# BigHippo123/pointcloud-raster

Measured on AMD Instinct MI355X. Metric: Mpts/s ingest->finalize, higher is better.
Workload: dtype f32

## Files before the change

pointcloud-raster_amd/csrc/engine.hip:

```cpp
#include "engine.hpp"

#include <cstdlib>
#include <map>
#include <mutex>
#include <new>
#include <vector>

using namespace pcrhip;

namespace {

struct SharedScratch {
    std::mutex borrow_mu;
    std::mutex mu;
    pcr_hip_arena* arena = nullptr;
    hipEvent_t last = nullptr;
    bool has_last = false;
    uint64_t borrows = 0, grows = 0;
    struct Taps {
        int K = -1, r = -1;
        float sx = 0.f, sy = 0.f;
        float* d = nullptr;
        size_t cap = 0;
        std::vector<float> host;
    } taps;
};
constexpr int kMaxDevices = 64;
SharedScratch g_scratch[kMaxDevices];

}

namespace pcrhip {

int ensure_scratch(pcr_hip_engine* e, size_t bytes) {
    PCR_REQUIRE(e->device >= 0 && e->device < kMaxDevices, "scratch: device ordinal out of range");
    SharedScratch& sp = g_scratch[e->device];
    const bool fresh = !e->scratch_borrowed;
    if (fresh) sp.borrow_mu.lock();
    std::lock_guard<std::mutex> lock(sp.mu);
    auto bail = [&](int rc) { if (fresh) sp.borrow_mu.unlock(); return rc; };
    if (!sp.last && hipEventCreateWithFlags(&sp.last, hipEventDisableTiming) != hipSuccess)
        return bail(fail(PCR_HIP_CUDA_ERROR, "scratch: cannot create the hand-over event"));
    size_t cap = 0;
    if (sp.arena) (void)pcr_hip_arena_stats(sp.arena, &cap, nullptr, nullptr);
    if (bytes > cap) {
        if (hipDeviceSynchronize() != hipSuccess) return bail(fail(PCR_HIP_CUDA_ERROR, "scratch: device synchronize failed"));
        if (sp.arena) (void)pcr_hip_arena_destroy(sp.arena);
        sp.arena = nullptr;
        sp.has_last = false;
        int rc = pcr_hip_arena_create(&sp.arena, bytes + bytes / 8);
        if (rc) return bail(rc);
        ++sp.grows;
    }
    void* base = nullptr;
    (void)pcr_hip_arena_reset(sp.arena);
    int rc = pcr_hip_arena_alloc(sp.arena, bytes, &base);
    if (rc) return bail(rc);
    if (fresh) {
        if (sp.has_last && hipStreamWaitEvent(e->stream, sp.last, 0) != hipSuccess)
            return bail(fail(PCR_HIP_CUDA_ERROR, "scratch: cannot order after the previous borrower"));
        ++sp.borrows;
    }
    (void)pcr_hip_arena_stats(sp.arena, &cap, nullptr, nullptr);
    e->d_scratch = static_cast<char*>(base);
    e->scratch_cap = cap;
    e->scratch_borrowed = true;
    return PCR_HIP_OK;
}

int shared_taps(pcr_hip_engine* e, int K, int r, float sx, float sy,
                void (*fill)(std::vector<float>&, int, int, float, float), const float** d_taps, size_t* count) {
    PCR_REQUIRE(e->scratch_borrowed, "shared_taps: the scratch must be borrowed");
    auto& t = g_scratch[e->device].taps;
    if (!(t.d && t.K == K && t.r == r && t.sx == sx && t.sy == sy)) {
        PCR_HIP_TRY(hipStreamSynchronize(e->stream));
        std::vector<float> next;
        fill(next, K, r, sx, sy);
        if (next.size() > t.cap) {
            PCR_HIP_TRY(hipDeviceSynchronize());
            if (t.d) (void)hipFree(t.d);
            t.d = nullptr;
            t.cap = 0;
            PCR_HIP_TRY(hipMalloc(reinterpret_cast<void**>(&t.d), next.size() * sizeof(float)));
            t.cap = next.size();
// ... 40 lines not shown

namespace {

struct DeviceGuard {
    int prev = -1;
    bool changed = false;
    explicit DeviceGuard(int dev) {
        if (hipGetDevice(&prev) == hipSuccess && prev != dev) changed = hipSetDevice(dev) == hipSuccess;
    }
    ~DeviceGuard() { if (changed) (void)hipSetDevice(prev); }
    DeviceGuard(const DeviceGuard&) = delete;
    DeviceGuard& operator=(const DeviceGuard&) = delete;
};

int check_planes(uint32_t mask, const pcr_hip_planes* p, uint32_t allowed, PlanesDev& out) {
    PCR_REQUIRE(p != nullptr, "scatter: null planes");
    PCR_REQUIRE(mask != 0 && (mask & ~allowed) == 0, "scatter: plane mask not supported for this glyph");
    PCR_REQUIRE(!(mask & PCR_HIP_PLANE_SUM) || p->d_sum, "scatter: SUM plane requested but d_sum is null");
    PCR_REQUIRE(!(mask & PCR_HIP_PLANE_WGT) || p->d_wgt, "scatter: WGT plane requested but d_wgt is null");
    PCR_REQUIRE(!(mask & PCR_HIP_PLANE_MAX) || p->d_max, "scatter: MAX plane requested but d_max is null");
    PCR_REQUIRE(!(mask & PCR_HIP_PLANE_MIN) || p->d_min, "scatter: MIN plane requested but d_min is null");
    out.sum = p->d_sum; out.wgt = p->d_wgt; out.mx = p->d_max; out.mn = p->d_min;
    return PCR_HIP_OK;
}

int begin_scatter(pcr_hip_engine* e, uint64_t n) {
    e->stats.points_in = n;
    e->stats.points_valid = 0;
    e->stats.lds_tile_w = e->stats.lds_tile_h = e->stats.lds_apron = e->stats.num_bins = 0;
    e->stats_scatter_chunk = 0;
    e->counters_published = false;
    return PCR_HIP_OK;
}

int begin_published(pcr_hip_engine* e) {
    if (!e->counters_clean) {
        PCR_HIP_TRY(hipMemsetAsync(e->d_counters, 0, 8 * sizeof(unsigned long long), e->stream));
        e->counters_clean = true;
    }
    e->publish_counters = true;
    return PCR_HIP_OK;
}

}

namespace pcrhip {

int fill_identity(pcr_hip_engine* e, uint32_t mask, const PlanesDev& pl) {
    ScopedKernelTimer t(e, "k_state_init");
    const int64_t cells = (int64_t)e->gd.st_rows * e->gd.W;
    int rc = PCR_HIP_OK;
    if ((mask & PCR_HIP_PLANE_SUM) && (rc = pcr_hip_plane_fill(pl.sum, 0.0f, cells, e->stream)) != PCR_HIP_OK) return rc;
    if ((mask & PCR_HIP_PLANE_WGT) && (rc = pcr_hip_plane_fill(pl.wgt, 0.0f, cells, e->stream)) != PCR_HIP_OK) return rc;
    if ((mask & PCR_HIP_PLANE_MAX) && (rc = pcr_hip_plane_fill(pl.mx, -FLT_MAX, cells, e->stream)) != PCR_HIP_OK) return rc;
    if ((mask & PCR_HIP_PLANE_MIN) && (rc = pcr_hip_plane_fill(pl.mn, FLT_MAX, cells, e->stream)) != PCR_HIP_OK) return rc;
    return rc;
}

}

extern "C" {

int pcr_hip_engine_create(pcr_hip_engine** out, const pcr_hip_grid* g, size_t scratch_bytes, pcr_hip_stream s) {
    PCR_REQUIRE(out, "engine_create: null out pointer");
    *out = nullptr;
    int rc = validate_grid(g);
    if (rc) return rc;
    auto* e = new (std::nothrow) pcr_hip_engine();
    if (!e) return fail(PCR_HIP_OUT_OF_MEMORY, "engine_create: host allocation failed");
    e->grid = *g;
    e->gd = make_grid_dev(*g);
    e->stream = static_cast<hipStream_t>(s);
    e->max_bins = kMaxBins;
    if (const char* dbg = std::getenv("PCR_HIP_DEBUG_MAX_BINS")) {
        const int v = std::atoi(dbg);
        if (v >= 1 && v < kMaxBins) e->max_bins = v;
    }
    if (const char* dbg = std::getenv("PCR_HIP_DEBUG_TWO_LEVEL")) e->two_level = std::atoi(dbg) != 0;
    hipError_t err = hipGetDevice(&e->device);
    hipDeviceProp_t prop;
    if (err == hipSuccess) err = hipGetDeviceProperties(&prop, e->device);
    if (err == hipSuccess) {
        e->num_cus = prop.multiProcessorCount > 0 ? prop.multiProcessorCount : 256;
        e->ntiles = e->gd.tiles_x * e->gd.tiles_y;
        err = hipMalloc(reinterpret_cast<void**>(&e->d_touched), (size_t)e->ntiles * sizeof(uint32_t));
    }
    const size_t count_bytes = ((size_t)kVirtualXcds * kMaxBins + kMaxTiles) * sizeof(unsigned);
    if (err == hipSuccess) err = hipMalloc(reinterpret_cast<void**>(&e->d_counters), 16 * sizeof(unsigned long long));
    if (err == hipSuccess) err = hipMalloc(reinterpret_cast<void**>(&e->d_bin_counts), count_bytes);
    if (err == hipSuccess) err = hipMemsetAsync(e->d_touched, 0, (size_t)e->ntiles * sizeof(uint32_t), e->stream);
    if (err == hipSuccess) err = hipMemsetAsync(e->d_counters, 0, 16 * sizeof(unsigned long long), e->stream);
    if (err == hipSuccess) err = hipMemsetAsync(e->d_bin_counts, 0, count_bytes, e->stream);
    e->counts_clean = e->counters_clean = err == hipSuccess;
    if (err == hipSuccess && scratch_bytes) {
        if (ensure_scratch(e, scratch_bytes) != PCR_HIP_OK) err = hipErrorOutOfMemory;
        else release_scratch(e);
    }
    if (err != hipSuccess) {
        std::string msg = std::string("engine_create: ") + hipGetErrorString(err);
        pcr_hip_engine_destroy(e);
        return fail(err == hipErrorOutOfMemory ? PCR_HIP_OUT_OF_MEMORY : PCR_HIP_CUDA_ERROR, msg);
    }
    *out = e;
    return PCR_HIP_OK;
}

int pcr_hip_engine_destroy(pcr_hip_engine* e) {
    if (!e) return PCR_HIP_OK;
    DeviceGuard dev(e->device);
    (void)hipStreamSynchronize(e->stream);
    for (auto& p : e->pending) { (void)hipEventDestroy(p.a); (void)hipEventDestroy(p.b); }
    if (e->d_touched) (void)hipFree(e->d_touched);
    if (e->d_counters) (void)hipFree(e->d_counters);
    if (e->d_bin_counts) (void)hipFree(e->d_bin_counts);
    delete e;
    return PCR_HIP_OK;
}

int pcr_hip_device_scratch_stats(int device, size_t* capacity, size_t* high_water, uint64_t* borrows, uint64_t* grows) {
    PCR_REQUIRE(device >= 0 && device < kMaxDevices, "device_scratch_stats: device ordinal out of range");
    SharedScratch& sp = g_scratch[device];
    std::lock_guard<std::mutex> lock(sp.mu);
    size_t cap = 0, hw = 0;
    if (sp.arena) (void)pcr_hip_arena_stats(sp.arena, &cap, nullptr, &hw);
    if (capacity) *capacity = cap;
    if (high_water) *high_water = hw;
    if (borrows) *borrows = sp.borrows;
    if (grows) *grows = sp.grows;
    return PCR_HIP_OK;
}

int pcr_hip_engine_set_path(pcr_hip_engine* e, int path) {
    PCR_REQUIRE(e, "engine_set_path: null engine");
    PCR_REQUIRE(path >= 0 && path <= 3,
                "engine_set_path: path must be 0 (auto), 1 (direct), 2 (binned) or 3 (moments, Gaussian only)");
    e->forced_path = path;
    return PCR_HIP_OK;
}

int pcr_hip_engine_planes_fresh(pcr_hip_engine* e, int fresh) {
    PCR_REQUIRE(e, "engine_planes_fresh: null engine");
    PCR_REQUIRE(fresh >= 0 && fresh <= 2, "engine_planes_fresh: 0 (accumulate), 1 (identity-filled) or 2 (undefined) expected");
    e->planes_fresh = fresh;
    return PCR_HIP_OK;
}

int pcr_hip_engine_finalize_with_scatter(pcr_hip_engine* e, int n_out, const int* rtypes, float* const* d_outs,
                                         uint32_t* d_bands_done) {
    PCR_REQUIRE(e, "engine_finalize_with_scatter: null engine");
    e->fused_outs.n = 0;
    e->fused_done = nullptr;
    if (n_out == 0) return PCR_HIP_OK;
    PCR_REQUIRE(rtypes && d_outs && d_bands_done, "engine_finalize_with_scatter: null argument");
    PCR_REQUIRE(n_out >= 1 && n_out <= PCR_HIP_MAX_FINALIZE_OUTPUTS, "engine_finalize_with_scatter: 1..8 outputs");
    for (int i = 0; i < n_out; ++i) {
        PCR_REQUIRE(rtypes[i] >= PCR_HIP_SUM && rtypes[i] <= PCR_HIP_COUNT, "pipeline: unknown reduction type");
        PCR_REQUIRE(d_outs[i] && (reinterpret_cast<uintptr_t>(d_outs[i]) & 15) == 0,
                    "engine_finalize_with_scatter: bands must be non-null and 16-byte aligned");
        e->fused_outs.rtype[i] = rtypes[i];
        e->fused_outs.out[i] = d_outs[i];
    }
    e->fused_outs.n = n_out;
    e->fused_done = d_bands_done;
    return PCR_HIP_OK;
}

// ... 200 lines not shown
```

pointcloud-raster_amd/csrc/engine.hpp:

```cpp
#pragma once

#include "common.hpp"

#include <functional>
#include <map>
#include <vector>

struct pcr_hip_engine {
    pcr_hip_grid grid{};
    pcrhip::GridDev gd{};
    hipStream_t stream = nullptr;
    int device = 0;
    int num_cus = 256;

    uint32_t* d_touched = nullptr;
    int ntiles = 0;
    unsigned long long* d_counters = nullptr;

    unsigned* d_bin_counts = nullptr;
    bool counts_clean = false;
    bool counters_clean = false;
    bool publish_counters = false;
    bool counters_published = false;

    int forced_path = 0;
    int max_bins = 0;
    int stats_scatter_chunk = 0;
    bool two_level = true;
    pcr_hip_scatter_stats stats{};
    int planes_fresh = 0;

    pcrhip::FinalizeOuts fused_outs{};
    uint32_t* fused_done = nullptr;
    bool fused_taken = false;

    bool profiling = false;
    std::string profile_only;
    struct Pending { const char* name; hipEvent_t a, b; };
    std::vector<Pending> pending;
    std::map<std::string, std::pair<uint32_t, double>> kernel_ms;

    char* d_scratch = nullptr;
    size_t scratch_cap = 0;
    bool scratch_borrowed = false;
};

namespace pcrhip {

int ensure_scratch(pcr_hip_engine* e, size_t bytes);
void allow_dynamic_lds(const pcr_hip_engine* e, const void* kernel, size_t bytes);
int zero_counters(pcr_hip_engine* e);
void release_scratch(pcr_hip_engine* e);
int shared_taps(pcr_hip_engine* e, int K, int r, float sx, float sy,
                void (*fill)(std::vector<float>&, int, int, float, float), const float** d_taps, size_t* count);

struct ScopedKernelTimer {
    pcr_hip_engine* e;
    const char* name;
    hipEvent_t a = nullptr, b = nullptr;
    ScopedKernelTimer(pcr_hip_engine* eng, const char* nm) : e(eng), name(nm) {
        if (!e->profiling) return;
        if (!e->profile_only.empty() && e->profile_only != nm) return;
        if (hipEventCreate(&a) != hipSuccess || hipEventCreate(&b) != hipSuccess) { a = b = nullptr; return; }
        (void)hipEventRecord(a, e->stream);
    }
    ~ScopedKernelTimer() {
        if (!a) return;
        (void)hipEventRecord(b, e->stream);
        e->pending.push_back({name, a, b});
    }
};

struct BinGeom {
    int tile_w, tile_h;
    int bins_x, bins_y, nbins;
    int chunk;
    int row0, rows;
    int sup_shift;
};
constexpr int kMaxBands = 32;
struct BinItem {
    unsigned bin, first, count, shared;
};
struct TailFill {
    const unsigned* n_items;
    void* plane[4];
    unsigned bits[4];
    long long n16;
};
struct BinBuffers {
    const uint2* records;
    const BinItem* items;
    const unsigned* n_items;
    int max_items;
    void* extra;
    bool fill_folded;
// ... 69 lines not shown
```

pointcloud-raster_amd/csrc/scatter_binned.hip:

```cpp
#include "engine.hpp"

#include <cstdlib>

using namespace pcrhip;

namespace {

constexpr int kThreads = 1024;
constexpr unsigned kLcellMask = (1u << kLcellBits) - 1;
constexpr unsigned kPointItemRecords = 1u << 17;

struct Routed {
    bool valid;
    int bin;
    unsigned lcell;
    int row, col;
};

__device__ __forceinline__ Routed route(const GridDev& g, const BinGeom& b, double wx, double wy) {
    Routed r;
    r.valid = world_to_cell(g, wx, wy, r.col, r.row);
    r.valid = r.valid && r.row >= g.own_r0 && r.row < g.own_r1;
    int sr = r.row - g.st_r0 - b.row0;
    int bx = fast_div(r.col, b.tile_w), by = fast_div(sr, b.tile_h);
// ... 386 lines not shown
    if (blockIdx.x >= *n_items) return;
    const BinItem it = items[blockIdx.x];
    const int tps = 1 << sup_shift;
    for (int i = threadIdx.x; i < tps; i += kThreads) lds_u32[i] = 0;
    __syncthreads();
    const unsigned tile0 = it.bin << sup_shift;
    const uint2* r = rec + it.first;
    for (unsigned j = threadIdx.x; j < it.count; j += kThreads) atomicAdd(&lds_u32[(r[j].x >> kLcellBits) - tile0], 1u);
    __syncthreads();
    for (int i = threadIdx.x; i < tps; i += kThreads) {
        const unsigned c = lds_u32[i];
        if (c) atomicAdd(&tile_count[tile0 + i], c);
    }
}

__global__ void __launch_bounds__(kThreads)
k_sub_scatter(int sup_shift, const uint2* __restrict__ rec, const BinItem* __restrict__ items,
              const unsigned* __restrict__ n_items, unsigned* __restrict__ cursor, uint2* __restrict__ out) {
    extern __shared__ unsigned char lds_raw[];
    if (blockIdx.x >= *n_items) return;
    const BinItem it = items[blockIdx.x];
    const int tps = 1 << sup_shift;
    uint2* stage = reinterpret_cast<uint2*>(lds_raw);
    unsigned* hist = reinterpret_cast<unsigned*>(lds_raw + (size_t)kSubPer * kThreads * sizeof(uint2));
    unsigned* loff = hist + tps;
    unsigned* gbase = loff + tps;
    __shared__ unsigned wave_tot[kThreads / 64];
    for (int i = threadIdx.x; i < tps; i += kThreads) hist[i] = 0;
    __syncthreads();
    const unsigned tile0 = it.bin << sup_shift;
    const uint2* r = rec + it.first;
    uint2 rc[kSubPer];
    unsigned rank[kSubPer];
#pragma unroll
    for (int k = 0; k < kSubPer; ++k) {
        const unsigned j = k * kThreads + threadIdx.x;
        rc[k] = j < it.count ? r[j] : make_uint2(0xFFFFFFFFu, 0u);
    }
#pragma unroll
    for (int k = 0; k < kSubPer; ++k) {
        rank[k] = 0;
        if (rc[k].x != 0xFFFFFFFFu) rank[k] = atomicAdd(&hist[(rc[k].x >> kLcellBits) - tile0], 1u);
    }
    __syncthreads();
    const int per = (tps + kThreads - 1) / kThreads;
    const int lo = threadIdx.x * per, hi = min(lo + per, tps);
    unsigned s = 0;
    for (int i = lo; i < hi; ++i) s += hist[i];
    unsigned incl = s;
    const int lane = threadIdx.x & 63, wave = threadIdx.x >> 6;
#pragma unroll
    for (int off = 1; off < 64; off <<= 1) {
        unsigned t = __shfl_up(incl, off, 64);
        if (lane >= off) incl += t;
    }
    if (lane == 63) wave_tot[wave] = incl;
    __syncthreads();
    unsigned run = incl - s;
    for (int w = 0; w < wave; ++w) run += wave_tot[w];
    for (int i = lo; i < hi; ++i) {
        loff[i] = run;
        run += hist[i];
    }
    for (int i = threadIdx.x; i < tps; i += kThreads) {
        const unsigned c = hist[i];
        if (c) gbase[i] = atomicAdd(&cursor[tile0 + i], c);
    }
    __syncthreads();
#pragma unroll
    for (int k = 0; k < kSubPer; ++k)
        if (rc[k].x != 0xFFFFFFFFu) stage[loff[(rc[k].x >> kLcellBits) - tile0] + rank[k]] = rc[k];
    __syncthreads();
    for (unsigned j = threadIdx.x; j < it.count; j += kThreads) {
        const uint2 q = stage[j];
        const unsigned t = (q.x >> kLcellBits) - tile0;
        out[gbase[t] + (j - loff[t])] = make_uint2(q.x & kLcellMask, q.y);
    }
}

inline int tile_cell_bytes(unsigned mask) {
    return ((mask & 1) ? 8 : 0) + ((mask & 2) ? 4 : 0) + ((mask & 4) ? 4 : 0) + ((mask & 8) ? 4 : 0);
}

inline BinGeom point_bin_geom(const GridDev& g, uint32_t mask) {
    BinGeom b{};
    b.tile_w = 128;
    b.tile_h = std::min(128, (150 * 1024 / (std::max(tile_cell_bytes(mask), 4) * 128)) & ~7);
    b.bins_x = (g.W + b.tile_w - 1) / b.tile_w;
    b.bins_y = (g.st_rows + b.tile_h - 1) / b.tile_h;
    b.nbins = b.bins_x * b.bins_y;
    b.rows = g.st_rows;
    return b;
}

template <unsigned MASK, bool FUSED>
__global__ void __launch_bounds__(kThreads)
k_tile_accum(GridDev g, BinGeom b, PlanesDev pl, const uint2* __restrict__ records,
             const BinItem* __restrict__ items, const unsigned* __restrict__ n_items, int fresh,
             FinalizeOuts fo, const uint32_t* __restrict__ touched, uint32_t* __restrict__ done) {
    extern __shared__ double lds_tile[];
    if (FUSED && blockIdx.x == 0 && threadIdx.x == 0) *done = (fresh == 2 && n_items[1] == 0u) ? 1u : 0u;
    if (blockIdx.x >= *n_items) return;
    const bool full = fresh == 2 && n_items[1] == 0u;
    const BinItem it = items[blockIdx.x];
    const int cells = b.tile_w * b.tile_h;
    double* t_sum = lds_tile;
    unsigned* t_wgt = reinterpret_cast<unsigned*>(t_sum + ((MASK & 1) ? cells : 0));
    float* t_max = reinterpret_cast<float*>(t_wgt + ((MASK & 2) ? cells : 0));
    float* t_min = t_max + ((MASK & 4) ? cells : 0);

    constexpr int kUnroll = 4;
    const uint2* rec = records + it.first;
    uint2 cur[kUnroll], nxt[kUnroll];
    auto fetch = [&](uint2 (&r)[kUnroll], unsigned j0) {
#pragma unroll
        for (int u = 0; u < kUnroll; ++u) {
            const unsigned j = j0 + u * kThreads;
            r[u] = j < it.count ? stream_load(rec + j) : make_uint2(0xFFFFFFFFu, 0u);
        }
    };
    fetch(cur, threadIdx.x);

    for (int i = threadIdx.x; i < cells; i += kThreads) {
        if (MASK & 1) t_sum[i] = 0.0;
        if (MASK & 2) t_wgt[i] = 0u;
        if (MASK & 4) t_max[i] = -FLT_MAX;
        if (MASK & 8) t_min[i] = FLT_MAX;
    }
    __syncthreads();

    for (unsigned j0 = threadIdx.x; j0 < it.count; j0 += kUnroll * kThreads) {
        fetch(nxt, j0 + kUnroll * kThreads);
#pragma unroll
        for (int u = 0; u < kUnroll; ++u) {
            if (cur[u].x == 0xFFFFFFFFu) continue;
            float val = __uint_as_float(cur[u].y);
            if (MASK & 1) unsafeAtomicAdd(&t_sum[cur[u].x], (double)val);
            if (MASK & 2) atomicAdd(&t_wgt[cur[u].x], 1u);
            if (MASK & 4) atomic_max_f32(&t_max[cur[u].x], val);
            if (MASK & 8) atomic_min_f32(&t_min[cur[u].x], val);
        }
#pragma unroll
        for (int u = 0; u < kUnroll; ++u) cur[u] = nxt[u];
    }
    __syncthreads();

    const int bx = it.bin % b.bins_x, by = it.bin / b.bins_x;
    const int c0 = bx * b.tile_w, r0 = b.row0 + by * b.tile_h;
    const int w = min(b.tile_w, g.W - c0), h = min(b.tile_h, b.row0 + b.rows - r0);
    const bool vec = !it.shared && (g.W % 4 == 0) && (w % 4 == 0) &&
                     ((((MASK & 1) ? reinterpret_cast<uintptr_t>(pl.sum) : 0) | ((MASK & 2) ? reinterpret_cast<uintptr_t>(pl.wgt) : 0) |
                       ((MASK & 4) ? reinterpret_cast<uintptr_t>(pl.mx) : 0) | ((MASK & 8) ? reinterpret_cast<uintptr_t>(pl.mn) : 0)) & 15) == 0;
    if (vec) {
        const int qrow = b.tile_w >> 2;
        for (int i = threadIdx.x; i < qrow * h; i += kThreads) {
            int ly = i / qrow, lx = (i - ly * qrow) << 2;
            if (lx >= w) continue;
            int64_t cell = (int64_t)(r0 + ly) * g.W + (c0 + lx);
            int li = ly * b.tile_w + lx;
            float4 a1, a2, a4, a8, g1, g2, g4, g8;
            bool n1 = false, n2 = false, n4 = false, n8 = false;
            if (MASK & 1) {
                double2 lo = *reinterpret_cast<const double2*>(t_sum + li), hi = *reinterpret_cast<const double2*>(t_sum + li + 2);
                a1 = make_float4((float)lo.x, (float)lo.y, (float)hi.x, (float)hi.y);
                n1 = (lo.x != 0.0) | (lo.y != 0.0) | (hi.x != 0.0) | (hi.y != 0.0);
            }
            if (MASK & 2) {
                uint4 c = *reinterpret_cast<const uint4*>(t_wgt + li);
                a2 = make_float4((float)c.x, (float)c.y, (float)c.z, (float)c.w);
                n2 = (c.x | c.y | c.z | c.w) != 0u;
            }
            if (MASK & 4) { a4 = *reinterpret_cast<const float4*>(t_max + li); n4 = (a4.x != -FLT_MAX) | (a4.y != -FLT_MAX) | (a4.z != -FLT_MAX) | (a4.w != -FLT_MAX); }
            if (MASK & 8) { a8 = *reinterpret_cast<const float4*>(t_min + li); n8 = (a8.x != FLT_MAX) | (a8.y != FLT_MAX) | (a8.z != FLT_MAX) | (a8.w != FLT_MAX); }
            if (fresh) {
                if (MASK & 1) g1 = make_float4(0.f, 0.f, 0.f, 0.f);
                if (MASK & 2) g2 = make_float4(0.f, 0.f, 0.f, 0.f);
                if (MASK & 4) g4 = make_float4(-FLT_MAX, -FLT_MAX, -FLT_MAX, -FLT_MAX);
                if (MASK & 8) g8 = make_float4(FLT_MAX, FLT_MAX, FLT_MAX, FLT_MAX);
            } else {
                if ((MASK & 1) && n1) g1 = *reinterpret_cast<const float4*>(pl.sum + cell);
                if ((MASK & 2) && n2) g2 = *reinterpret_cast<const float4*>(pl.wgt + cell);
                if ((MASK & 4) && n4) g4 = *reinterpret_cast<const float4*>(pl.mx + cell);
                if ((MASK & 8) && n8) g8 = *reinterpret_cast<const float4*>(pl.mn + cell);
            }
            typedef float f4v __attribute__((ext_vector_type(4)));
            if (full) n1 = n2 = n4 = n8 = true;
            if ((MASK & 1) && n1) { g1.x += a1.x; g1.y += a1.y; g1.z += a1.z; g1.w += a1.w;
                __builtin_nontemporal_store(f4v{g1.x, g1.y, g1.z, g1.w}, reinterpret_cast<f4v*>(pl.sum + cell)); }
            if ((MASK & 2) && n2) { g2.x += a2.x; g2.y += a2.y; g2.z += a2.z; g2.w += a2.w;
                __builtin_nontemporal_store(f4v{g2.x, g2.y, g2.z, g2.w}, reinterpret_cast<f4v*>(pl.wgt + cell)); }
            if ((MASK & 4) && n4) { g4.x = fmaxf(g4.x, a4.x); g4.y = fmaxf(g4.y, a4.y); g4.z = fmaxf(g4.z, a4.z); g4.w = fmaxf(g4.w, a4.w); *reinterpret_cast<float4*>(pl.mx + cell) = g4; }
            if ((MASK & 8) && n8) { g8.x = fminf(g8.x, a8.x); g8.y = fminf(g8.y, a8.y); g8.z = fminf(g8.z, a8.z); g8.w = fminf(g8.w, a8.w); *reinterpret_cast<float4*>(pl.mn + cell) = g8; }
            if (FUSED && full) {
                const float s4[4] = {g1.x, g1.y, g1.z, g1.w}, w4[4] = {g2.x, g2.y, g2.z, g2.w};
                const float x4[4] = {g4.x, g4.y, g4.z, g4.w}, m4[4] = {g8.x, g8.y, g8.z, g8.w};
                const int trow = ((g.st_r0 + r0 + ly) / g.th) * g.tiles_x;
                bool live[4];
#pragma unroll
                for (int k = 0; k < 4; ++k) live[k] = touched[trow + (c0 + lx + k) / g.tw] != 0u;
                for (int o = 0; o < fo.n; ++o) {
                    float v[4];
#pragma unroll
                    for (int k = 0; k < 4; ++k)
                        v[k] = live[k] ? finalize_rt(fo.rtype[o], (MASK & 1) ? s4[k] : 0.f, (MASK & 2) ? w4[k] : 0.f,
                                                     (MASK & 4) ? x4[k] : -FLT_MAX, (MASK & 8) ? m4[k] : FLT_MAX) : NAN;
                    __builtin_nontemporal_store(f4v{v[0], v[1], v[2], v[3]}, reinterpret_cast<f4v*>(fo.out[o] + cell));
                }
            }
        }
        return;
    }
    for (int i = threadIdx.x; i < b.tile_w * h; i += kThreads) {
        int ly = i / b.tile_w, lx = i - ly * b.tile_w;
        if (lx >= w) continue;
        int64_t cell = (int64_t)(r0 + ly) * g.W + (c0 + lx);
        int li = ly * b.tile_w + lx;
        if (full) {
            if (MASK & 1) pl.sum[cell] = (float)t_sum[li];
            if (MASK & 2) pl.wgt[cell] = (float)t_wgt[li];
            if (MASK & 4) pl.mx[cell] = t_max[li];
            if (MASK & 8) pl.mn[cell] = t_min[li];
        } else if (!it.shared) {
            if (MASK & 1) { double a = t_sum[li]; if (a != 0.0) pl.sum[cell] += (float)a; }
            if (MASK & 2) { unsigned a = t_wgt[li]; if (a) pl.wgt[cell] += (float)a; }
            if (MASK & 4) { float a = t_max[li]; if (a != -FLT_MAX) pl.mx[cell] = fmaxf(pl.mx[cell], a); }
            if (MASK & 8) { float a = t_min[li]; if (a != FLT_MAX) pl.mn[cell] = fminf(pl.mn[cell], a); }
        } else {
            if (MASK & 1) { double a = t_sum[li]; if (a != 0.0) atomic_add_f32(pl.sum + cell, (float)a); }
            if (MASK & 2) { unsigned a = t_wgt[li]; if (a) atomic_add_f32(pl.wgt + cell, (float)a); }
            if (MASK & 4) { float a = t_max[li]; if (a != -FLT_MAX) atomic_max_f32(pl.mx + cell, a); }
            if (MASK & 8) { float a = t_min[li]; if (a != FLT_MAX) atomic_min_f32(pl.mn + cell, a); }
        }
    }
}

__global__ void __launch_bounds__(256)
k_fill_if(const unsigned* __restrict__ n_items, PlanesDev pl, unsigned mask, int64_t cells4) {
    if (n_items[1] == 0u) return;
    const float4 zero = make_float4(0.f, 0.f, 0.f, 0.f), lo = make_float4(-FLT_MAX, -FLT_MAX, -FLT_MAX, -FLT_MAX),
                 hi = make_float4(FLT_MAX, FLT_MAX, FLT_MAX, FLT_MAX);
    const int64_t stride = (int64_t)gridDim.x * 256;
    for (int64_t i = (int64_t)blockIdx.x * 256 + threadIdx.x; i < cells4; i += stride) {
        if (mask & 1) reinterpret_cast<float4*>(pl.sum)[i] = zero;
        if (mask & 2) reinterpret_cast<float4*>(pl.wgt)[i] = zero;
        if (mask & 4) reinterpret_cast<float4*>(pl.mx)[i] = lo;
        if (mask & 8) reinterpret_cast<float4*>(pl.mn)[i] = hi;
    }
}

template <unsigned MASK>
void launch_accum(pcr_hip_engine* e, const GridDev& gd, const BinGeom& b, const PlanesDev& pl, const BinBuffers& bb,
                  bool fused = false) {
    size_t lds = (size_t)b.tile_w * b.tile_h * tile_cell_bytes(MASK);
    auto go = [&](auto kernel, const FinalizeOuts& fo, uint32_t* done) {
        allow_dynamic_lds(e, reinterpret_cast<const void*>(kernel), lds);
        hipLaunchKernelGGL(kernel, dim3(bb.max_items), dim3(kThreads), lds, e->stream, gd, b, pl,
                           bb.records, bb.items, bb.n_items, e->planes_fresh, fo, (const uint32_t*)e->d_touched, done);
    };
    if (fused) go(&k_tile_accum<MASK, true>, e->fused_outs, e->fused_done);
    else go(&k_tile_accum<MASK, false>, FinalizeOuts{}, nullptr);
}

constexpr uint32_t kSelectGeomMask = PCR_HIP_PLANE_SUM;

__global__ void __launch_bounds__(kThreads)
k_tile_select(GridDev g, BinGeom b, unsigned long long* __restrict__ packed, const uint2* __restrict__ records,
              const BinItem* __restrict__ items, const unsigned* __restrict__ n_items, int fresh,
              const unsigned long long* __restrict__ words) {
    extern __shared__ unsigned long long lds_words[];
    if (blockIdx.x >= *n_items) return;
    const bool full = fresh == 2 && n_items[1] == 0u;
    const BinItem it = items[blockIdx.x];
    const int cells = b.tile_w * b.tile_h;

    constexpr int kUnroll = 4;
    const uint2* rec = records + it.first;
    uint2 cur[kUnroll], nxt[kUnroll];
    auto fetch = [&](uint2 (&r)[kUnroll], unsigned j0) {
#pragma unroll
        for (int u = 0; u < kUnroll; ++u) {
            const unsigned j = j0 + u * kThreads;
            r[u] = j < it.count ? stream_load(rec + j) : make_uint2(0xFFFFFFFFu, 0u);
        }
    };
    fetch(cur, threadIdx.x);
    for (int i = threadIdx.x; i < cells; i += kThreads) lds_words[i] = 0ull;
    __syncthreads();

    for (unsigned j0 = threadIdx.x; j0 < it.count; j0 += kUnroll * kThreads) {
        fetch(nxt, j0 + kUnroll * kThreads);
        unsigned long long w[kUnroll];
#pragma unroll
        for (int u = 0; u < kUnroll; ++u) w[u] = cur[u].x != 0xFFFFFFFFu ? words[cur[u].y] : 0ull;
#pragma unroll
        for (int u = 0; u < kUnroll; ++u)
            if (w[u]) atomicMax(&lds_words[cur[u].x], w[u]);
#pragma unroll
        for (int u = 0; u < kUnroll; ++u) cur[u] = nxt[u];
    }
    __syncthreads();

    const int bx = it.bin % b.bins_x, by = it.bin / b.bins_x;
    const int c0 = bx * b.tile_w, r0 = b.row0 + by * b.tile_h;
    const int w = min(b.tile_w, g.W - c0), h = min(b.tile_h, b.row0 + b.rows - r0);
    const bool vec = !it.shared && (g.W % 2 == 0) && (w % 2 == 0) && (reinterpret_cast<uintptr_t>(packed) & 15) == 0;
    if (vec) {
        const int hrow = b.tile_w >> 1;
        for (int i = threadIdx.x; i < hrow * h; i += kThreads) {
            const int ly = i / hrow, lx = (i - ly * hrow) << 1;
            if (lx >= w) continue;
            ulonglong2* dst = reinterpret_cast<ulonglong2*>(packed + (int64_t)(r0 + ly) * g.W + (c0 + lx));
            ulonglong2 a = *reinterpret_cast<const ulonglong2*>(lds_words + ly * b.tile_w + lx);
            if (!full && !(a.x | a.y)) continue;
            if (!fresh) {
                const ulonglong2 cur2 = *dst;
                a.x = a.x > cur2.x ? a.x : cur2.x;
                a.y = a.y > cur2.y ? a.y : cur2.y;
            }
            *dst = a;
        }
        return;
    }
    for (int i = threadIdx.x; i < b.tile_w * h; i += kThreads) {
        const int ly = i / b.tile_w, lx = i - ly * b.tile_w;
        if (lx >= w) continue;
        unsigned long long* dst = packed + (int64_t)(r0 + ly) * g.W + (c0 + lx);
        const unsigned long long a = lds_words[ly * b.tile_w + lx];
        if (full) *dst = a;
        else if (!a) continue;
        else if (it.shared) atomicMax(dst, a);
        else if (fresh) *dst = a;
        else if (a > *dst) *dst = a;
    }
}

template <bool VEC>
// ... 110 lines not shown
    if (rc) return rc;
    char* s = e->d_scratch;
    auto U = [&](size_t o) { return reinterpret_cast<unsigned*>(s + o); };
    BinItem* d_items1 = reinterpret_cast<BinItem*>(s + o_items1);
    uint2* d_rec1 = reinterpret_cast<uint2*>(s + o_rec1);
    PCR_REQUIRE(l1.nbins <= kMaxBins && (!shift || b.nbins <= kMaxTiles), "bin_points: more bins than the count arrays hold");
    unsigned* const d_count1 = e->d_bin_counts;
    unsigned* const d_count2 = e->d_bin_counts + (size_t)nvx * kMaxBins;
    auto scan = [&](int nbins, int vx, unsigned records, unsigned* d_count, size_t o_cursor, size_t o_items, size_t o_nitems, bool every,
                    int publish) {
        ScopedKernelTimer t(e, "k_bin_scan");
        hipLaunchKernelGGL(k_bin_scan, dim3(1), dim3(kThreads), 0, e->stream, nbins, vx, records, d_count, U(o_cursor),
                           reinterpret_cast<BinItem*>(s + o_items), U(o_nitems), every ? 1 : 0, e->d_counters, publish);
    };
    if (!e->counts_clean)
        PCR_HIP_TRY(hipMemsetAsync(e->d_bin_counts, 0, ((size_t)nvx * kMaxBins + kMaxTiles) * sizeof(unsigned), e->stream));
    e->counts_clean = false;
    const int publish = !e->publish_counters ? 0 : e->counters_published ? 2 : 1;
    if (publish) e->counters_clean = false;
    TailFill tf{};
    if (fill && !shift) {
        tf = *fill;
        tf.n_items = U(o_nitems1);
    }
    launch_count(e, gd, l1, full_blocks, x, y, n, U(o_keys), d_count1);
    scan(l1.nbins, nvx, item_records1, d_count1, o_cursor1, o_items1, o_nitems1, every_bin && !shift, publish);
    if (index) launch_bin_scatter<true>(e, l1, nvx, U(o_keys), v, n, U(o_cursor1), d_rec1, tf);
    else launch_bin_scatter<false>(e, l1, nvx, U(o_keys), v, n, U(o_cursor1), d_rec1, tf);
    if (shift) {
        const int tps = 1 << shift;
        {
            ScopedKernelTimer t(e, "k_sub_count");
            hipLaunchKernelGGL(k_sub_count, dim3(max_items1), dim3(kThreads), (size_t)tps * 4, e->stream, shift,
                               d_rec1, d_items1, U(o_nitems1), d_count2);
        }
        scan(b.nbins, 1, item_records, d_count2, o_cursor2, o_items2, o_nitems2, every_bin, 0);
        ScopedKernelTimer t(e, "k_sub_scatter");
        const size_t lds = (size_t)sub_records * sizeof(uint2) + (size_t)tps * 4 * 3;
        allow_dynamic_lds(e, reinterpret_cast<const void*>(&k_sub_scatter), lds);
        hipLaunchKernelGGL(k_sub_scatter, dim3(max_items1), dim3(kThreads), lds, e->stream, shift, d_rec1, d_items1,
                           U(o_nitems1), U(o_cursor2), reinterpret_cast<uint2*>(s + o_rec2));
    }
    PCR_HIP_TRY(hipGetLastError());
    e->counts_clean = true;
    if (publish) e->counters_clean = e->counters_published = true;
    out->fill_folded = tf.n_items != nullptr;
    out->records = reinterpret_cast<uint2*>(s + (shift ? o_rec2 : o_rec1));
    out->items = reinterpret_cast<BinItem*>(s + (shift ? o_items2 : o_items1));
    out->n_items = U(shift ? o_nitems2 : o_nitems1);
    out->max_items = max_items;
    out->extra = extra_bytes ? s + o_extra : nullptr;
    return PCR_HIP_OK;
}

int sweep_passes(const pcr_hip_engine* e, const BinGeom& whole) { return plan_sweep(e, whole).passes; }

int sweep_tiles(pcr_hip_engine* e, const BinGeom& whole, const double* x, const double* y, const float* v, uint64_t n,
                RecordKind kind, unsigned item_records, bool every_bin, size_t extra_bytes, const TilePass& tile_pass,
                const TailFill* fill) {
    const SweepPlan plan = plan_sweep(e, whole);
    if (plan.passes < 1) return -fail(PCR_HIP_INVALID_ARGUMENT, "binned scatter: grid cannot be binned");
    int total_bins = 0;
    for (int pass = 0; pass < plan.passes; ++pass) {
        const int row0 = pass * plan.band_rows, rows = std::min(plan.band_rows, e->gd.st_rows - row0);
        const GridDev gd = band_grid(e->gd, row0, rows);
        if (gd.own_r0 >= gd.own_r1 && !plan.shift) continue;
        BinGeom b = whole;
        b.row0 = row0;
        b.rows = rows;
        b.bins_y = (rows + b.tile_h - 1) / b.tile_h;
        b.nbins = b.bins_x * b.bins_y;
        b.sup_shift = plan.shift;
        total_bins += b.nbins;
        BinBuffers bb{};
        int rc = bin_points(e, gd, b, x, y, v, n, kind, item_records, &bb, every_bin, extra_bytes, fill);
        if (rc == PCR_HIP_OK) rc = tile_pass(gd, b, bb);
        if (rc) return -rc;
    }
    return total_bins;
}

bool binned_point_supported(const pcr_hip_engine* e, uint32_t mask) {
    if (mask == 0 || (mask & ~15u)) return false;
    if (sweep_passes(e, point_bin_geom(e->gd, mask)) < 1) return false;
    uint64_t cells = (uint64_t)e->gd.W * e->gd.st_rows;
    if (e->forced_path != 2 && e->stats.points_in * 16 < cells) return false;
    return e->stats.points_in < (1ull << 32) - (1ull << 20);
}

int binned_point(pcr_hip_engine* e, uint32_t mask, const PlanesDev& pl,
                 const double* x, const double* y, const float* v, uint64_t n) {
    const BinGeom whole = point_bin_geom(e->gd, mask);
    const int64_t cells = (int64_t)e->gd.st_rows * e->gd.W;
    const bool define_all = e->planes_fresh == 2 && sweep_passes(e, whole) == 1 && cells % 4 == 0 &&
                            ((reinterpret_cast<uintptr_t>(pl.sum) | reinterpret_cast<uintptr_t>(pl.wgt) |
                              reinterpret_cast<uintptr_t>(pl.mx) | reinterpret_cast<uintptr_t>(pl.mn)) & 15) == 0;
    if (e->planes_fresh == 2 && !define_all) {
        int rc = fill_identity(e, mask, pl);
        if (rc) return rc;
        e->planes_fresh = 1;
    }
    const bool fused = define_all && e->fused_outs.n > 0 && e->fused_done && e->gd.W % 4 == 0 &&
                       e->gd.own_r0 == e->gd.st_r0 && e->gd.own_r1 - e->gd.own_r0 == e->gd.st_rows;
    TailFill fill{};
    fill.plane[0] = (mask & 1) ? pl.sum : nullptr; fill.bits[0] = 0u;
    fill.plane[1] = (mask & 2) ? pl.wgt : nullptr; fill.bits[1] = 0u;
    fill.plane[2] = (mask & 4) ? pl.mx : nullptr;  fill.bits[2] = 0xFF7FFFFFu;
    fill.plane[3] = (mask & 8) ? pl.mn : nullptr;  fill.bits[3] = 0x7F7FFFFFu;
    fill.n16 = cells / 4;
    const int bins = sweep_tiles(e, whole, x, y, v, n, RecordKind::Value, kPointItemRecords, define_all, 0,
                                 [&](const GridDev& gd, const BinGeom& b, const BinBuffers& bb) {
        if (define_all && !bb.fill_folded)
            hipLaunchKernelGGL(k_fill_if, dim3(2048), dim3(256), 0, e->stream, bb.n_items, pl, mask, cells / 4);
        e->fused_taken = fused;
        ScopedKernelTimer t(e, "k_tile_accum");
        switch (mask) {
#define PCR_ACC(M) case M: launch_accum<M>(e, gd, b, pl, bb, fused); break;
            PCR_ACC(1) PCR_ACC(2) PCR_ACC(3) PCR_ACC(4) PCR_ACC(5) PCR_ACC(6) PCR_ACC(7) PCR_ACC(8)
            PCR_ACC(9) PCR_ACC(10) PCR_ACC(11) PCR_ACC(12) PCR_ACC(13) PCR_ACC(14) PCR_ACC(15)
#undef PCR_ACC
            default: return fail(PCR_HIP_INVALID_ARGUMENT, "scatter_point: empty plane mask");
        }
        return (int)PCR_HIP_OK;
    }, define_all ? &fill : nullptr);
    if (bins < 0) return -bins;
    PCR_HIP_TRY(hipGetLastError());
    set_binned_stats(e, 1, whole.tile_w, whole.tile_h, 0, bins);
    return PCR_HIP_OK;
}

bool binned_select_supported(const pcr_hip_engine* e) { return binned_point_supported(e, kSelectGeomMask); }

int binned_select(pcr_hip_engine* e, unsigned long long* packed, const double* x, const double* y, const float* v,
                  const float* key, uint64_t n) {
    const BinGeom whole = point_bin_geom(e->gd, kSelectGeomMask);
    const int64_t cells = (int64_t)e->gd.st_rows * e->gd.W;
    const bool define_all = e->planes_fresh == 2 && sweep_passes(e, whole) == 1 && cells % 2 == 0 && e->gd.W % 2 == 0 &&
                            (reinterpret_cast<uintptr_t>(packed) & 15) == 0;
    if (e->planes_fresh == 2 && !define_all) {
        ScopedKernelTimer t(e, "k_state_init");
        PCR_HIP_TRY(hipMemsetAsync(packed, 0, (size_t)cells * sizeof(unsigned long long), e->stream));
        e->planes_fresh = 1;
    }
    TailFill fill{};
    fill.plane[0] = packed;
    fill.n16 = cells / 2;
    const int bins = sweep_tiles(e, whole, x, y, nullptr, n, RecordKind::Index, kPointItemRecords, define_all, (size_t)n * 8,
                                 [&](const GridDev& gd, const BinGeom& b, const BinBuffers& bb) {
        if (define_all && !bb.fill_folded)
            hipLaunchKernelGGL(k_zero_if, dim3(2048), dim3(256), 0, e->stream, bb.n_items, packed, cells / 2);
        launch_select(e, gd, b, packed, bb, v, key, n);
        return (int)PCR_HIP_OK;
    }, define_all ? &fill : nullptr);
    if (bins < 0) return -bins;
    PCR_HIP_TRY(hipGetLastError());
    set_binned_stats(e, 1, whole.tile_w, whole.tile_h, 0, bins);
    return PCR_HIP_OK;
}

}
```

Before: 96840.

## Size point tiles to CU count and precompute tile liveness in fused accumulate

Point-bin tile height is now picked by searching heights that minimise rounds-per-CU times height, bounded by the device LDS limit read at engine creation. The fused accumulate kernel gets a dedicated fast path for fresh full bins. It writes planes directly without reading global memory, and it computes per-tile touched flags once through a wave ballot, or through an LDS bitmask when a tile is mixed, instead of per-cell global lookups. Finalize outputs are produced with a branch-free select in place of a per-output finalize_rt call. Taller tiles use more LDS, which may reduce occupancy.

```diff
diff --git a/pointcloud-raster_amd/csrc/engine.hip b/pointcloud-raster_amd/csrc/engine.hip
--- a/pointcloud-raster_amd/csrc/engine.hip
+++ b/pointcloud-raster_amd/csrc/engine.hip
@@ -1,5 +1,6 @@
 #include "engine.hpp"
 
+#include <algorithm>
 #include <cstdlib>
 #include <map>
 #include <mutex>
@@ -206,6 +207,7 @@
     if (err == hipSuccess) err = hipGetDeviceProperties(&prop, e->device);
     if (err == hipSuccess) {
         e->num_cus = prop.multiProcessorCount > 0 ? prop.multiProcessorCount : 256;
+        e->lds_limit = std::max(prop.sharedMemPerBlock, prop.sharedMemPerBlockOptin);
         e->ntiles = e->gd.tiles_x * e->gd.tiles_y;
         err = hipMalloc(reinterpret_cast<void**>(&e->d_touched), (size_t)e->ntiles * sizeof(uint32_t));
     }
diff --git a/pointcloud-raster_amd/csrc/engine.hpp b/pointcloud-raster_amd/csrc/engine.hpp
--- a/pointcloud-raster_amd/csrc/engine.hpp
+++ b/pointcloud-raster_amd/csrc/engine.hpp
@@ -12,6 +12,7 @@
     hipStream_t stream = nullptr;
     int device = 0;
     int num_cus = 256;
+    size_t lds_limit = 64 * 1024;
 
     uint32_t* d_touched = nullptr;
     int ntiles = 0;
diff --git a/pointcloud-raster_amd/csrc/scatter_binned.hip b/pointcloud-raster_amd/csrc/scatter_binned.hip
--- a/pointcloud-raster_amd/csrc/scatter_binned.hip
+++ b/pointcloud-raster_amd/csrc/scatter_binned.hip
@@ -492,11 +492,26 @@
     return ((mask & 1) ? 8 : 0) + ((mask & 2) ? 4 : 0) + ((mask & 4) ? 4 : 0) + ((mask & 8) ? 4 : 0);
 }
 
-inline BinGeom point_bin_geom(const GridDev& g, uint32_t mask) {
+constexpr int kPointTileW = 128;
+inline size_t point_tile_lds(int bytes_per_cell, int h) { return (size_t)kPointTileW * h * bytes_per_cell + (size_t)kPointTileW * h / 8; }
+
+inline BinGeom point_bin_geom(const pcr_hip_engine* e, uint32_t mask) {
+    const GridDev& g = e->gd;
+    const int bytes = std::max(tile_cell_bytes(mask), 4);
     BinGeom b{};
-    b.tile_w = 128;
-    b.tile_h = std::min(128, (150 * 1024 / (std::max(tile_cell_bytes(mask), 4) * 128)) & ~7);
+    b.tile_w = kPointTileW;
     b.bins_x = (g.W + b.tile_w - 1) / b.tile_w;
+    auto bins_of = [&](int h) { return (int64_t)b.bins_x * ((g.st_rows + h - 1) / h); };
+    auto rounds_of = [&](int h) { return (bins_of(h) + e->num_cus - 1) / e->num_cus; };
+    b.tile_h = std::min(128, (150 * 1024 / (bytes * kPointTileW)) & ~7);
+    if (rounds_of(b.tile_h) <= 16) {
+        int64_t best = rounds_of(b.tile_h) * b.tile_h;
+        for (int h = b.tile_h + 8; kPointTileW * h <= (1 << kLcellBits) && point_tile_lds(bytes, h) <= e->lds_limit; h += 8)
+            if (rounds_of(h) * h < best) {
+                best = rounds_of(h) * h;
+                b.tile_h = h;
+            }
+    }
     b.bins_y = (g.st_rows + b.tile_h - 1) / b.tile_h;
     b.nbins = b.bins_x * b.bins_y;
     b.rows = g.st_rows;
@@ -513,11 +528,15 @@
     if (blockIdx.x >= *n_items) return;
     const bool full = fresh == 2 && n_items[1] == 0u;
     const BinItem it = items[blockIdx.x];
-    const int cells = b.tile_w * b.tile_h;
+    const int cells = kPointTileW * b.tile_h;
     double* t_sum = lds_tile;
     unsigned* t_wgt = reinterpret_cast<unsigned*>(t_sum + ((MASK & 1) ? cells : 0));
     float* t_max = reinterpret_cast<float*>(t_wgt + ((MASK & 2) ? cells : 0));
     float* t_min = t_max + ((MASK & 4) ? cells : 0);
+    unsigned* t_live = reinterpret_cast<unsigned*>(t_min + ((MASK & 8) ? cells : 0));
+    const int bx = it.bin % b.bins_x, by = it.bin / b.bins_x;
+    const int c0 = bx * kPointTileW, r0 = b.row0 + by * b.tile_h;
+    const int w = min(kPointTileW, g.W - c0), h = min(b.tile_h, b.row0 + b.rows - r0);
 
     constexpr int kUnroll = 4;
     const uint2* rec = records + it.first;
@@ -530,12 +549,48 @@
         }
     };
     fetch(cur, threadIdx.x);
+
+    unsigned live_all = 0xFu, flag = 0u;
+    bool live_mixed = false;
+    int nt = 0;
+    if (FUSED && full) {
+        const int tr0 = (g.st_r0 + r0) / g.th, tc0 = c0 / g.tw;
+        const int nc = (c0 + w - 1) / g.tw - tc0 + 1, lane = threadIdx.x & 63;
+        nt = ((g.st_r0 + r0 + h - 1) / g.th - tr0 + 1) * nc;
+        if (nt <= 64 && lane < nt) flag = touched[(tr0 + lane / nc) * g.tiles_x + tc0 + lane % nc];
+    }
 
     for (int i = threadIdx.x; i < cells; i += kThreads) {
         if (MASK & 1) t_sum[i] = 0.0;
         if (MASK & 2) t_wgt[i] = 0u;
         if (MASK & 4) t_max[i] = -FLT_MAX;
         if (MASK & 8) t_min[i] = FLT_MAX;
+    }
+
+    if (FUSED && full) {
+        asm volatile("" : "+v"(flag));
+        live_mixed = nt > 64;
+        if (!live_mixed) {
+            const int set = __popcll(__ballot(flag != 0u));
+            live_all = set == nt ? 0xFu : 0u;
+            live_mixed = set != 0 && set != nt;
+        }
+        if (live_mixed)
+            for (int t = threadIdx.x; t < cells / 32; t += kThreads) {
+                const int ly = t >> 2, cb = c0 + ((t & 3) << 5);
+                unsigned bits = 0u;
+                if (ly < h && cb < g.W) {
+                    const uint32_t* trow = touched + ((g.st_r0 + r0 + ly) / g.th) * g.tiles_x;
+                    int tc = cb / g.tw, next = (tc + 1) * g.tw;
+                    unsigned on = trow[tc] != 0u;
+                    const int n = min(32, g.W - cb);
+                    for (int k = 0; k < n; ++k) {
+                        if (cb + k >= next) { ++tc; next += g.tw; on = trow[tc] != 0u; }
+                        bits |= on << k;
+                    }
+                }
+                t_live[t] = bits;
+            }
     }
     __syncthreads();
 
@@ -555,19 +610,98 @@
     }
     __syncthreads();
 
-    const int bx = it.bin % b.bins_x, by = it.bin / b.bins_x;
-    const int c0 = bx * b.tile_w, r0 = b.row0 + by * b.tile_h;
-    const int w = min(b.tile_w, g.W - c0), h = min(b.tile_h, b.row0 + b.rows - r0);
     const bool vec = !it.shared && (g.W % 4 == 0) && (w % 4 == 0) &&
                      ((((MASK & 1) ? reinterpret_cast<uintptr_t>(pl.sum) : 0) | ((MASK & 2) ? reinterpret_cast<uintptr_t>(pl.wgt) : 0) |
                        ((MASK & 4) ? reinterpret_cast<uintptr_t>(pl.mx) : 0) | ((MASK & 8) ? reinterpret_cast<uintptr_t>(pl.mn) : 0)) & 15) == 0;
+    typedef float f4v __attribute__((ext_vector_type(4)));
+    const int lx = (threadIdx.x & 31) << 2, ly0 = threadIdx.x >> 5;
+    if (vec && full) {
+        if (lx >= w || ly0 >= h) return;
+        const int n_out = FUSED ? fo.n : 0;
+        float* band[PCR_HIP_MAX_FINALIZE_OUTPUTS];
+        bool divides = false;
+        unsigned kinds = 0u;
+#pragma unroll
+        for (int o = 0; o < PCR_HIP_MAX_FINALIZE_OUTPUTS; ++o) {
+            band[o] = fo.out[o];
+            kinds |= ((unsigned)fo.rtype[o] & 7u) << (3 * o);
+            divides |= o < n_out && (fo.rtype[o] == PCR_HIP_AVERAGE || fo.rtype[o] == PCR_HIP_WEIGHTED_AVERAGE);
+        }
+        const unsigned vkinds = (unsigned)vector_resident((int)kinds);
+        struct Quad {
+            double2 slo, shi;
+            uint4 cnt;
+            float4 mx, mn;
+            unsigned live;
+        };
+        auto read = [&](int ly) {
+            Quad q{};
+            const int li = ly * kPointTileW + lx;
+            if (MASK & 1) { q.slo = *reinterpret_cast<const double2*>(t_sum + li); q.shi = *reinterpret_cast<const double2*>(t_sum + li + 2); }
+            if (MASK & 2) q.cnt = *reinterpret_cast<const uint4*>(t_wgt + li);
+            if (MASK & 4) q.mx = *reinterpret_cast<const float4*>(t_max + li);
+            if (MASK & 8) q.mn = *reinterpret_cast<const float4*>(t_min + li);
+            q.live = live_all;
+            if (FUSED && live_mixed) q.live = t_live[li >> 5];
+            return q;
+        };
+        const int live_shift = (FUSED && live_mixed) ? (lx & 31) : 0;
+        Quad nq = read(ly0);
+        int64_t cell = (int64_t)(r0 + ly0) * g.W + (c0 + lx);
+        for (int ly = ly0; ly < h; ly += 32, cell += (int64_t)32 * g.W) {
+            const Quad q = nq;
+            if (ly + 32 < h) nq = read(ly + 32);
+            float s4[4] = {0.f, 0.f, 0.f, 0.f}, w4[4] = {0.f, 0.f, 0.f, 0.f};
+            float x4[4] = {-FLT_MAX, -FLT_MAX, -FLT_MAX, -FLT_MAX}, m4[4] = {FLT_MAX, FLT_MAX, FLT_MAX, FLT_MAX};
+            if (MASK & 1) { s4[0] += (float)q.slo.x; s4[1] += (float)q.slo.y; s4[2] += (float)q.shi.x; s4[3] += (float)q.shi.y; }
+            if (MASK & 2) { w4[0] += (float)q.cnt.x; w4[1] += (float)q.cnt.y; w4[2] += (float)q.cnt.z; w4[3] += (float)q.cnt.w; }
+            if (MASK & 4) { x4[0] = fmaxf(x4[0], q.mx.x); x4[1] = fmaxf(x4[1], q.mx.y); x4[2] = fmaxf(x4[2], q.mx.z); x4[3] = fmaxf(x4[3], q.mx.w); }
+            if (MASK & 8) { m4[0] = fminf(m4[0], q.mn.x); m4[1] = fminf(m4[1], q.mn.y); m4[2] = fminf(m4[2], q.mn.z); m4[3] = fminf(m4[3], q.mn.w); }
+            float cnt4[4], avg4[4], max4[4], min4[4];
+            if (FUSED) {
+#pragma unroll
+                for (int k = 0; k < 4; ++k) {
+                    cnt4[k] = w4[k] > 0.0f ? w4[k] : NAN;
+                    avg4[k] = NAN;
+                    max4[k] = x4[k] == -FLT_MAX ? NAN : x4[k];
+                    min4[k] = m4[k] == FLT_MAX ? NAN : m4[k];
+                }
+                if (divides) {
+#pragma unroll
+                    for (int k = 0; k < 4; ++k) avg4[k] = w4[k] > 0.0f ? s4[k] / w4[k] : NAN;
+                }
+            }
+            if (MASK & 1) __builtin_nontemporal_store(f4v{s4[0], s4[1], s4[2], s4[3]}, reinterpret_cast<f4v*>(pl.sum + cell));
+            if (MASK & 2) __builtin_nontemporal_store(f4v{w4[0], w4[1], w4[2], w4[3]}, reinterpret_cast<f4v*>(pl.wgt + cell));
+            if (MASK & 4) *reinterpret_cast<float4*>(pl.mx + cell) = make_float4(x4[0], x4[1], x4[2], x4[3]);
+            if (MASK & 8) *reinterpret_cast<float4*>(pl.mn + cell) = make_float4(m4[0], m4[1], m4[2], m4[3]);
+            if (FUSED) {
+#pragma unroll
+                for (int o = 0; o < PCR_HIP_MAX_FINALIZE_OUTPUTS; ++o) {
+                    if (o >= n_out) break;
+                    const unsigned kind = (vkinds >> (3 * o)) & 7u;
+                    const bool is_sum = kind == PCR_HIP_SUM, is_cnt = kind == PCR_HIP_COUNT, is_max = kind == PCR_HIP_MAX, is_min = kind == PCR_HIP_MIN;
+                    float v[4];
+#pragma unroll
+                    for (int k = 0; k < 4; ++k) {
+                        float f = avg4[k];
+                        f = is_min ? min4[k] : f;
+                        f = is_max ? max4[k] : f;
+                        f = is_cnt ? cnt4[k] : f;
+                        f = is_sum ? s4[k] : f;
+                        v[k] = ((q.live >> (live_shift + k)) & 1u) ? f : NAN;
+                    }
+                    __builtin_nontemporal_store(f4v{v[0], v[1], v[2], v[3]}, reinterpret_cast<f4v*>(band[o] + cell));
+                }
+            }
+        }
+        return;
+    }
     if (vec) {
-        const int qrow = b.tile_w >> 2;
-        for (int i = threadIdx.x; i < qrow * h; i += kThreads) {
-            int ly = i / qrow, lx = (i - ly * qrow) << 2;
-            if (lx >= w) continue;
+        if (lx >= w) return;
+        for (int ly = ly0; ly < h; ly += 32) {
             int64_t cell = (int64_t)(r0 + ly) * g.W + (c0 + lx);
-            int li = ly * b.tile_w + lx;
+            int li = ly * kPointTileW + lx;
             float4 a1, a2, a4, a8, g1, g2, g4, g8;
             bool n1 = false, n2 = false, n4 = false, n8 = false;
             if (MASK & 1) {
@@ -593,30 +727,12 @@
                 if ((MASK & 4) && n4) g4 = *reinterpret_cast<const float4*>(pl.mx + cell);
                 if ((MASK & 8) && n8) g8 = *reinterpret_cast<const float4*>(pl.mn + cell);
             }
-            typedef float f4v __attribute__((ext_vector_type(4)));
-            if (full) n1 = n2 = n4 = n8 = true;
             if ((MASK & 1) && n1) { g1.x += a1.x; g1.y += a1.y; g1.z += a1.z; g1.w += a1.w;
                 __builtin_nontemporal_store(f4v{g1.x, g1.y, g1.z, g1.w}, reinterpret_cast<f4v*>(pl.sum + cell)); }
             if ((MASK & 2) && n2) { g2.x += a2.x; g2.y += a2.y; g2.z += a2.z; g2.w += a2.w;
                 __builtin_nontemporal_store(f4v{g2.x, g2.y, g2.z, g2.w}, reinterpret_cast<f4v*>(pl.wgt + cell)); }
             if ((MASK & 4) && n4) { g4.x = fmaxf(g4.x, a4.x); g4.y = fmaxf(g4.y, a4.y); g4.z = fmaxf(g4.z, a4.z); g4.w = fmaxf(g4.w, a4.w); *reinterpret_cast<float4*>(pl.mx + cell) = g4; }
             if ((MASK & 8) && n8) { g8.x = fminf(g8.x, a8.x); g8.y = fminf(g8.y, a8.y); g8.z = fminf(g8.z, a8.z); g8.w = fminf(g8.w, a8.w); *reinterpret_cast<float4*>(pl.mn + cell) = g8; }
-            if (FUSED && full) {
-                const float s4[4] = {g1.x, g1.y, g1.z, g1.w}, w4[4] = {g2.x, g2.y, g2.z, g2.w};
-                const float x4[4] = {g4.x, g4.y, g4.z, g4.w}, m4[4] = {g8.x, g8.y, g8.z, g8.w};
-                const int trow = ((g.st_r0 + r0 + ly) / g.th) * g.tiles_x;
-                bool live[4];
-#pragma unroll
-                for (int k = 0; k < 4; ++k) live[k] = touched[trow + (c0 + lx + k) / g.tw] != 0u;
-                for (int o = 0; o < fo.n; ++o) {
-                    float v[4];
-#pragma unroll
-                    for (int k = 0; k < 4; ++k)
-                        v[k] = live[k] ? finalize_rt(fo.rtype[o], (MASK & 1) ? s4[k] : 0.f, (MASK & 2) ? w4[k] : 0.f,
-                                                     (MASK & 4) ? x4[k] : -FLT_MAX, (MASK & 8) ? m4[k] : FLT_MAX) : NAN;
-                    __builtin_nontemporal_store(f4v{v[0], v[1], v[2], v[3]}, reinterpret_cast<f4v*>(fo.out[o] + cell));
-                }
-            }
         }
         return;
     }
@@ -661,7 +777,7 @@
 template <unsigned MASK>
 void launch_accum(pcr_hip_engine* e, const GridDev& gd, const BinGeom& b, const PlanesDev& pl, const BinBuffers& bb,
                   bool fused = false) {
-    size_t lds = (size_t)b.tile_w * b.tile_h * tile_cell_bytes(MASK);
+    const size_t lds = fused ? point_tile_lds(tile_cell_bytes(MASK), b.tile_h) : (size_t)b.tile_w * b.tile_h * tile_cell_bytes(MASK);
     auto go = [&](auto kernel, const FinalizeOuts& fo, uint32_t* done) {
         allow_dynamic_lds(e, reinterpret_cast<const void*>(kernel), lds);
         hipLaunchKernelGGL(kernel, dim3(bb.max_items), dim3(kThreads), lds, e->stream, gd, b, pl,
@@ -938,7 +1054,7 @@
 
 bool binned_point_supported(const pcr_hip_engine* e, uint32_t mask) {
     if (mask == 0 || (mask & ~15u)) return false;
-    if (sweep_passes(e, point_bin_geom(e->gd, mask)) < 1) return false;
+    if (sweep_passes(e, point_bin_geom(e, mask)) < 1) return false;
     uint64_t cells = (uint64_t)e->gd.W * e->gd.st_rows;
     if (e->forced_path != 2 && e->stats.points_in * 16 < cells) return false;
     return e->stats.points_in < (1ull << 32) - (1ull << 20);
@@ -946,7 +1062,7 @@
 
 int binned_point(pcr_hip_engine* e, uint32_t mask, const PlanesDev& pl,
                  const double* x, const double* y, const float* v, uint64_t n) {
-    const BinGeom whole = point_bin_geom(e->gd, mask);
+    const BinGeom whole = point_bin_geom(e, mask);
     const int64_t cells = (int64_t)e->gd.st_rows * e->gd.W;
     const bool define_all = e->planes_fresh == 2 && sweep_passes(e, whole) == 1 && cells % 4 == 0 &&
                             ((reinterpret_cast<uintptr_t>(pl.sum) | reinterpret_cast<uintptr_t>(pl.wgt) |
@@ -989,7 +1105,7 @@
 
 int binned_select(pcr_hip_engine* e, unsigned long long* packed, const double* x, const double* y, const float* v,
                   const float* key, uint64_t n) {
-    const BinGeom whole = point_bin_geom(e->gd, kSelectGeomMask);
+    const BinGeom whole = point_bin_geom(e, kSelectGeomMask);
     const int64_t cells = (int64_t)e->gd.st_rows * e->gd.W;
     const bool define_all = e->planes_fresh == 2 && sweep_passes(e, whole) == 1 && cells % 2 == 0 && e->gd.W % 2 == 0 &&
                             (reinterpret_cast<uintptr_t>(packed) & 15) == 0;
```

Result: faster. 99800 (median of 6 runs) (+3.1%).
